# minyoungpark1/Speech-Enhancement

Hardware: AMD Instinct MI355X
Metric: utterances/sec (2 s @16 kHz) CMGAN train step (higher is better)
Workload: dtype f32 (f16x3 split); 1 GPU; cmgan generator+discriminator train step (main_gan.py train_gan loop body), batch 16/GPU, 2 s @ 16 kHz, n_fft=400 hop=100, AdamW lr 5e-4, PESQ labels supplied, kaiming-init weights; fp32 results throughout: conv and token GEMMs as scaled fp16 hi/lo splits (3 MFMAs per product, 2^-24 relative, fp32 accumulate), attention on the same scaled fp16 splits (scales from measured operand maxima), everythi; global_batch=16, parallelism=dp1

## Files before the change

speech-enhancement_amd/csrc/se_gemm.hip:

```cpp

#include "se_gemm_dev.h"


template <int BK, int PRO, bool LIN>
__global__ __launch_bounds__(256) void gemm_tap_kernel(GemmArgs g) {
  constexpr int BM = 128, BN = 64, SA = BK + 4;
  constexpr int KQ = BK / 4;
  constexpr int RPP = 256 / KQ;
  constexpr int NA = BM / RPP, NB = BN / RPP;
  __shared__ __attribute__((aligned(16))) float As[BM * SA];
  __shared__ __attribute__((aligned(16))) float Bs[BN * SA];
  __shared__ float red[4 * 64 * 2];
  __shared__ __attribute__((aligned(16))) float bias_s[64];

  const se_gemm_desc& d = g.d;
  const int tid = threadIdx.x, lane = tid & 63, wave = tid >> 6;
  const WorkId wk_ = decode_work(g.ncb, g.nouter, g.contig);
  if (wk_.outer >= g.nouter) return;
  const int b = wk_.outer / g.tiles, by = wk_.inner;
  const int Mb = d.To * d.Fo;
  const int m0 = (wk_.outer - b * g.tiles) * BM;
  const bool glu = (d.epilogue & SE_EPI_GLU) != 0;
  const int kq = tid % KQ, r0 = tid / KQ;
  constexpr bool lin = LIN;
// ... 853 lines not shown
    vr[3][ks][0] = *reinterpret_cast<const float4*>(cp + 64); vr[3][ks][1] = *reinterpret_cast<const float4*>(cp + 68);
  };
  if (k0 < ntile) {
#pragma unroll
    for (int ks = 0; ks < 4; ++ks) request(k0, ks);
  }
  int b_staged = -1;
  for (int kk = k0; kk < ntile; kk += gx) {
    const int tile = xbase + kk;
    const int b = tile / g.tiles, m0 = (tile - b * g.tiles) * 128;
    const bool ok = row_ok(kk);
    if (b != b_staged) {
      __syncthreads();
      ss_s[tid] = g.ps[(long)b * 256 + tid];
      __syncthreads();
      b_staged = b;
    }
    f32x16 acc[4];
#pragma unroll
    for (int c = 0; c < 4; ++c)
#pragma unroll
      for (int r = 0; r < 16; ++r) acc[c][r] = 0.f;
#pragma unroll
    for (int ks = 0; ks < 4; ++ks) {
      asm volatile("" ::: "memory");
      float x[8];
      {
        const float gr[8] = {vr[0][ks][0].x, vr[0][ks][0].y, vr[0][ks][0].z, vr[0][ks][0].w, vr[0][ks][1].x, vr[0][ks][1].y, vr[0][ks][1].z, vr[0][ks][1].w};
        const float fr[8] = {vr[1][ks][0].x, vr[1][ks][0].y, vr[1][ks][0].z, vr[1][ks][0].w, vr[1][ks][1].x, vr[1][ks][1].y, vr[1][ks][1].z, vr[1][ks][1].w};
        const float cg[8] = {vr[2][ks][0].x, vr[2][ks][0].y, vr[2][ks][0].z, vr[2][ks][0].w, vr[2][ks][1].x, vr[2][ks][1].y, vr[2][ks][1].z, vr[2][ks][1].w};
        const float cf[8] = {vr[3][ks][0].x, vr[3][ks][0].y, vr[3][ks][0].z, vr[3][ks][0].w, vr[3][ks][1].x, vr[3][ks][1].y, vr[3][ks][1].z, vr[3][ks][1].w};
        const float* sg = ss_s + 2 * (16 * ks + 8 * kg);
#pragma unroll
        for (int j = 0; j < 8; j += 2) {
          const float4 pg = *reinterpret_cast<const float4*>(sg + 2 * j), pf = *reinterpret_cast<const float4*>(sg + 128 + 2 * j);
          const float zg0 = fmaf(gr[j], pg.x, pg.y) + cg[j], zg1 = fmaf(gr[j + 1], pg.z, pg.w) + cg[j + 1];
          const float zf0 = fmaf(fr[j], pf.x, pf.y) + cf[j], zf1 = fmaf(fr[j + 1], pf.z, pf.w) + cf[j + 1];
          const float t0 = 1.0f - 2.0f * __builtin_amdgcn_rcpf(1.0f + __builtin_amdgcn_exp2f(2.8853900817779268f * zf0));
          const float t1 = 1.0f - 2.0f * __builtin_amdgcn_rcpf(1.0f + __builtin_amdgcn_exp2f(2.8853900817779268f * zf1));
          x[j] = ok ? sigmoidf_(zg0) * t0 : 0.f;
          x[j + 1] = ok ? sigmoidf_(zg1) * t1 : 0.f;
        }
      }
      bf16x8 af[2];
      split_planes8_h(x, sa, af);
#ifdef SE_GATE_PROJ_EARLY
      if (ks < 2) request(kk + gx, ks);
#endif
#pragma unroll
      for (int cb = 0; cb < 2; ++cb) {
        bf16x8 bf0[2], bf1[2];
#pragma unroll
        for (int pl = 0; pl < 2; ++pl) {
          bf0[pl] = *reinterpret_cast<const bf16x8*>(&Wl[(cb * 2 + pl) * PW + frag + 16 * ks]);
          bf1[pl] = *reinterpret_cast<const bf16x8*>(&Wl[(cb * 2 + pl) * PW + 32 * SW + frag + 16 * ks]);
        }
        acc[2 * cb] = mfma32_<true>(af[1], bf0[0], acc[2 * cb]); acc[2 * cb + 1] = mfma32_<true>(af[1], bf1[0], acc[2 * cb + 1]);
        acc[2 * cb] = mfma32_<true>(af[0], bf0[1], acc[2 * cb]); acc[2 * cb + 1] = mfma32_<true>(af[0], bf1[1], acc[2 * cb + 1]);
        acc[2 * cb] = mfma32_<true>(af[0], bf0[0], acc[2 * cb]); acc[2 * cb + 1] = mfma32_<true>(af[0], bf1[0], acc[2 * cb + 1]);
      }
    }
#pragma unroll
    for (int c = 0; c < 4; ++c)
#pragma unroll
      for (int r = 0; r < 16; ++r) acc[c][r] *= unscale;
#pragma unroll
    for (int cb = 0; cb < 2; ++cb) {
      gemm_epilogue_vec<false, false, true>(g, acc[2 * cb], acc[2 * cb + 1], m0, cb, b, cs, 36, 0u, 1.f, red, bias_s + 64 * cb, {}, &ymax);
      if (d.epilogue & SE_EPI_STATS) __syncthreads();
    }
#ifndef SE_GATE_PROJ_EARLY
    request(kk + gx, 0);
    request(kk + gx, 1);
#endif
    request(kk + gx, 2);
    request(kk + gx, 3);
  }
  if (g.amax_out) {
    ymax = wave_max(ymax);
    if ((threadIdx.x & 63) == 0) amax_raise_(g.amax_out, ymax);
  }
}

template <int PRO>
__global__ __launch_bounds__(512, 1) void gemm_k64_wstat_kernel(GemmArgs g) {
  constexpr int SB = 72;
  extern __shared__ __attribute__((aligned(16))) unsigned char smem_ws[];
  const se_gemm_desc& d = g.d;
  const int tid = threadIdx.x, lane = tid & 63, wave = tid >> 6;
  const int Mb = d.To * d.Fo;
  float ymax = 0.f;
  const int ncb = g.ncb, NR = ncb * 64, PB = NR * SB;
  __bf16* Bp = reinterpret_cast<__bf16*>(smem_ws);
  float* patch = reinterpret_cast<float*>(smem_ws + (size_t)2 * PB * 2);
  float* pss = patch + 8 * 32 * 36;
  float* bias_all = pss + 128;
  const bool glu = (d.epilogue & SE_EPI_GLU) != 0;
  const unsigned thr = drop_thr(d.drop_p);
  const float inv_keep = drop_inv_keep(d.drop_p);
  f16_clamp_mode_();
  const int ea = operand_sexp_(d.a_amax, d.a_sexp), ew = operand_sexp_(d.w_amax, d.w_sexp);
  const float sa = exp2i_(ea), unscale = exp2i_(-ea - ew);
  for (int i = tid; i < NR * 8; i += 512) {
    const int j = i >> 3, ch = i & 7, by = j >> 6, jl = j & 63;
    int n; bool ok;
    if (glu) { n = (jl >> 5) * (d.N / 2) + by * 32 + (jl & 31); ok = (by * 32 + (jl & 31)) < d.N / 2; }
    else { n = j; ok = n < d.N; }
    const __bf16* wp = reinterpret_cast<const __bf16*>(g.W) + ((unsigned)(ok ? n : 0) * (unsigned)d.ldw + 8 * ch);
#pragma unroll
    for (int q = 0; q < 2; ++q) {
      const uint4 w4 = *reinterpret_cast<const uint4*>(wp + (size_t)q * (size_t)d.w_planes);
      *reinterpret_cast<uint4*>(&Bp[q * PB + j * SB + 8 * ch]) = make_uint4(ok ? w4.x : 0u, ok ? w4.y : 0u, ok ? w4.z : 0u, ok ? w4.w : 0u);
    }
  }
  if (PRO == SE_PRO_LN && tid < 32) *reinterpret_cast<float4*>(&pss[4 * tid]) = *reinterpret_cast<const float4*>((tid < 16 ? g.ps : g.pb - 64) + 4 * tid);
  for (int i = tid; i < NR; i += 512) {
    const int by = i >> 6, jl = i & 63;
    int n; bool ok;
    if (glu) { n = (jl >> 5) * (d.N / 2) + by * 32 + (jl & 31); ok = (by * 32 + (jl & 31)) < d.N / 2; }
    else { n = i; ok = n < d.N; }
    bias_all[i] = ((d.epilogue & SE_EPI_BIAS) && ok) ? g.bias[n] : 0.f;
  }
  __syncthreads();
  const bool vec_ep = epilogue_vec_ok(d);
  const int kg = lane >> 5;
  const int frag = (lane & 31) * SB + 8 * kg;
  float* cs = patch + wave * 32 * 36;
  const int ntile = (Mb + 255) / 256;
  float4 v[4][2];
  float2 mr = make_float2(0.f, 0.f);
  auto request = [&](int tile) {
    const int row = tile * 256 + wave * 32 + (lane & 31);
    const long rowl = row < Mb ? row : Mb - 1;
    const float* __restrict__ ap = g.A + rowl * d.lda + d.a_off + 8 * kg;
    if (PRO == SE_PRO_LN) mr = *reinterpret_cast<const float2*>(g.rowstats + 2 * rowl);
#pragma unroll
    for (int ks = 0; ks < 4; ++ks) {
      v[ks][0] = *reinterpret_cast<const float4*>(ap + 16 * ks);
      v[ks][1] = *reinterpret_cast<const float4*>(ap + 16 * ks + 4);
    }
  };
  if ((int)blockIdx.x < ntile) request(blockIdx.x);
  for (int tile = blockIdx.x; tile < ntile; tile += gridDim.x) {
    const int m0 = tile * 256;
    const int row = m0 + wave * 32 + (lane & 31);
    const bool rok = row < Mb;
    bf16x8 af[4][2];
#pragma unroll
    for (int ks = 0; ks < 4; ++ks) {
      float x[8];
#pragma unroll
      for (int h = 0; h < 2; ++h) {
        const int c = 16 * ks + 8 * kg + 4 * h;
        float4 w = v[ks][h];
        if (PRO == SE_PRO_LN)
          w = apply_pro<PRO>(w, c, 64, mr.x, mr.y, *reinterpret_cast<const float4*>(&pss[c]), *reinterpret_cast<const float4*>(&pss[64 + c]),
                             (unsigned)row, d.pro_seed, thr, inv_keep);
        x[4 * h] = rok ? w.x : 0.f; x[4 * h + 1] = rok ? w.y : 0.f; x[4 * h + 2] = rok ? w.z : 0.f; x[4 * h + 3] = rok ? w.w : 0.f;
      }
      split_planes8_h(x, sa, af[ks]);
    }
    if (tile + (int)gridDim.x < ntile) request(tile + gridDim.x);
    for (int by = 0; by < ncb; ++by) {
      f32x16 acc0, acc1;
#pragma unroll
      for (int r = 0; r < 16; ++r) { acc0[r] = 0.f; acc1[r] = 0.f; }
      const __bf16* Bb = Bp + by * 64 * SB;
#pragma unroll
      for (int ks = 0; ks < 4; ++ks) {
        bf16x8 bf0[2], bf1[2];
#pragma unroll
        for (int pl = 0; pl < 2; ++pl) {
          bf0[pl] = *reinterpret_cast<const bf16x8*>(&Bb[pl * PB + frag + 16 * ks]);
          bf1[pl] = *reinterpret_cast<const bf16x8*>(&Bb[pl * PB + 32 * SB + frag + 16 * ks]);
        }
        acc0 = mfma32_<true>(af[ks][0], bf0[1], acc0); acc1 = mfma32_<true>(af[ks][0], bf1[1], acc1);
        acc0 = mfma32_<true>(af[ks][1], bf0[0], acc0); acc1 = mfma32_<true>(af[ks][1], bf1[0], acc1);
        acc0 = mfma32_<true>(af[ks][0], bf0[0], acc0); acc1 = mfma32_<true>(af[ks][0], bf1[0], acc1);
      }
#pragma unroll
      for (int r = 0; r < 16; ++r) { acc0[r] *= unscale; acc1[r] *= unscale; }
      if (vec_ep) gemm_epilogue_vec<false, false, true>(g, acc0, acc1, m0, by, 0, cs, 36, thr, inv_keep, nullptr, bias_all + by * 64, {}, &ymax);
      else gemm_epilogue_glu_vec(g, acc0, acc1, m0, by, 0, cs, 36, bias_all + by * 64);
    }
  }
  if (g.amax_out) {
    ymax = wave_max(ymax);
    if ((threadIdx.x & 63) == 0) amax_raise_(g.amax_out, ymax);
  }
}

__global__ void repack_kernel(const float* src, float* dst, int No, int Nt, int Ni, long so, long stt,
                              long si, int rev, int accumulate) {
  long idx = (long)blockIdx.x * blockDim.x + threadIdx.x;
  long total = (long)No * Nt * Ni;
  if (idx >= total) return;
  int i = (int)(idx % Ni);
  int t = (int)((idx / Ni) % Nt);
  int o = (int)(idx / ((long)Ni * Nt));
  int is = i, os = o;
  if (rev == 1) { int ns = Ni / 64; is = (ns - 1 - i / 64) * 64 + (i & 63); }
  if (rev == 2) { int ns = No / 64; os = (ns - 1 - o / 64) * 64 + (o & 63); }
  float v = src[os * so + is * si + t * stt];
  if (accumulate) dst[idx] += v; else dst[idx] = v;
}

__global__ void unpack_kernel(const float* src, float* dst, int No, int Nt, int Ni, long so, long stt,
                              long si, int rev, int accumulate) {
  long idx = (long)blockIdx.x * blockDim.x + threadIdx.x;
  long total = (long)No * Nt * Ni;
  if (idx >= total) return;
  int i = (int)(idx % Ni);
  int t = (int)((idx / Ni) % Nt);
  int o = (int)(idx / ((long)Ni * Nt));
  int is = i, os = o;
  if (rev == 1) { int ns = Ni / 64; is = (ns - 1 - i / 64) * 64 + (i & 63); }
  if (rev == 2) { int ns = No / 64; os = (ns - 1 - o / 64) * 64 + (o & 63); }
  float* p = &dst[os * so + is * si + t * stt];
  if (accumulate) *p += src[idx]; else *p = src[idx];
}

extern "C" int se_gemm_tap(const se_gemm_desc* d, const float* A, const float* W, const float* bias,
                           float* Y, const float* R, float* AUX, const float* rowstats,
                           const float* pro_scale, const float* pro_shift, double* stats, void* stream) {
  if (int e = check_desc(d)) return e;
  const int ep = d->epilogue;
  SE_REQUIRE(!(ep & SE_EPI_LN_BWD_), "gemm: unknown epilogue bit 1024 (use se_gemm_ln_bwd)");
  SE_REQUIRE(A && W && Y, "gemm: null operand");
  SE_REQUIRE(!(ep & SE_EPI_BIAS) || bias, "gemm: bias flag without bias");
  SE_REQUIRE(!(ep & SE_EPI_RESID) || R, "gemm: resid flag without R");
  SE_REQUIRE(!(ep & SE_EPI_SWISH_GRAD) || AUX, "gemm: swish-grad flag without AUX");
  SE_REQUIRE(!(ep & SE_EPI_STATS) || stats, "gemm: stats flag without buffer");
  if (ep & SE_EPI_ROWSTATS)
    SE_REQUIRE(AUX && d->N == 64 && d->C >= 32 && d->ntap == 1 && d->B == 1 && !(ep & (SE_EPI_GLU | SE_EPI_SHUFFLE2 | SE_EPI_SWISH_GRAD | SE_EPI_STATS)) &&
               (d->ldc & 3) == 0 && (d->c_off & 3) == 0 && (d->ldr & 3) == 0 && (d->r_off & 3) == 0,
               "gemm: SE_EPI_ROWSTATS needs a row GEMM with N == 64, AUX = [M][2] and a vector-epilogue layout");
  if (ep & SE_EPI_DELTA)
    SE_REQUIRE(AUX && R && d->N == 64 && d->C >= 32 && d->ntap == 1 && d->B == 1 &&
               !(ep & (SE_EPI_GLU | SE_EPI_SHUFFLE2 | SE_EPI_SWISH_GRAD | SE_EPI_STATS | SE_EPI_RESID | SE_EPI_ROWSTATS | SE_EPI_ACCUM | 256)) &&
               (d->ldc & 3) == 0 && (d->c_off & 3) == 0 && d->ldr >= 64 && (d->ldr & 3) == 0 && (d->r_off & 3) == 0,
               "gemm: SE_EPI_DELTA needs a row GEMM with C >= 32, N == 64, R = O [M][64], AUX = [M][4] and a vector-epilogue layout");
  SE_REQUIRE(!(ep & (SE_EPI_GLU | SE_EPI_SHUFFLE2)) || (d->N % 2) == 0, "gemm: GLU/shuffle need even N");
  SE_REQUIRE(!(ep & SE_EPI_GLU_GATE) || ((ep & SE_EPI_GLU) && AUX), "gemm: SE_EPI_GLU_GATE needs SE_EPI_GLU and AUX");
  if (d->prologue == SE_PRO_LN) SE_REQUIRE(rowstats && pro_scale && pro_shift, "gemm: LN prologue operands");
  if (d->prologue == SE_PRO_AFFINE_SWISH) SE_REQUIRE(pro_scale && pro_shift, "gemm: affine prologue operands");
  if (d->precision == 3)
    SE_REQUIRE(d->C >= 32 && (!d->w_planes || d->w_amax), "gemm: precision 3 (scaled split-fp16) needs C >= 32; pre-split planes need w_amax");
  if (d->w_planes) {
    SE_REQUIRE((d->precision == 2 || d->precision == 3) && d->C >= 32 && (d->C % 8) == 0 && (d->ldw % 8) == 0 && d->w_planes >= (long)d->N * d->ldw &&
               (d->w_planes % 8) == 0 && ((size_t)W & 15) == 0,
               "gemm: pre-split weights need precision 2, C >= 32, C, ldw and the plane stride multiples of 8, a 16-byte aligned W");
    SE_REQUIRE((long)d->w_planes * 6 < (1L << 31), "gemm: pre-split weight planes exceed 2^31 bytes");
  }
  GemmArgs g{*d, A, W, bias, Y, R, AUX, rowstats, pro_scale, pro_shift, stats, nullptr, nullptr, 0, 0, 0, 0};
  g.amax_out = d->y_amax;
  SE_REQUIRE(!d->y_amax || (!(ep & (SE_EPI_GLU | SE_EPI_SHUFFLE2 | 256)) && (d->N & 3) == 0 && (d->ldc & 3) == 0 && (d->c_off & 3) == 0 &&
                            (d->ldx & 3) == 0 && (d->x_off & 3) == 0 && (d->ldr & 3) == 0 && (d->r_off & 3) == 0),
             "gemm: y_amax needs the vector epilogue (no GLU / shuffle, 4-aligned strides)");
  const int Mb = d->To * d->Fo;
  const int ncols = (ep & SE_EPI_GLU) ? cdiv(d->N / 2, 32) : cdiv(d->N, 64);
  g.ncb = ncols;
  g.tiles = cdiv(Mb, 128);
  g.nouter = d->B * g.tiles;
  g.contig = d->ntap > 1;
  dim3 grid((unsigned)(ncols * (((long)g.nouter + 7) / 8 * 8))), block(256);
  const bool lin = d->ntap == 1 && !d->up && d->st == 1 && d->sf == 1 && d->dt[0] == 0 && d->df[0] == 0 &&
                   d->Ti == d->To && d->Fi == d->Fo;
  hipStream_t s = as_stream(stream);
  {
    const bool vec_ok = !(ep & (SE_EPI_GLU | SE_EPI_SHUFFLE2 | SE_EPI_STATS | 256)) && (d->N & 3) == 0 && (d->ldc & 3) == 0 &&
                        (d->c_off & 3) == 0 && (d->ldx & 3) == 0 && (d->x_off & 3) == 0 && (d->ldr & 3) == 0 && (d->r_off & 3) == 0;
    const bool glu_ok = (ep & SE_EPI_GLU) && !(ep & (SE_EPI_STATS | SE_EPI_SHUFFLE2 | SE_EPI_DROP | SE_EPI_RESID | SE_EPI_ACCUM |
                                                       SE_EPI_SWISH_GRAD | 256)) &&
                        (d->N & 7) == 0 && (d->ldc & 3) == 0 && (d->c_off & 3) == 0 && (d->ldx & 3) == 0 && (d->x_off & 3) == 0;
    const bool map1d = d->To == 1 && d->Ti == 1 && d->Fi == d->Fo && d->st == 1 && d->sf == 1 && !d->up;
    const bool vec_st = vec_ok || ((ep & SE_EPI_STATS) && map1d && !(ep & (SE_EPI_GLU | SE_EPI_SHUFFLE2 | SE_EPI_ROWSTATS | 256)) &&
                                   (d->N & 3) == 0 && (d->ldc & 3) == 0 && (d->c_off & 3) == 0 && (d->ldx & 3) == 0 &&
                                   (d->x_off & 3) == 0 && (d->ldr & 3) == 0 && (d->r_off & 3) == 0);
    const bool tap3 = map1d && d->ntap == 3 && d->dt[0] == 0 && d->dt[1] == 0 && d->dt[2] == 0 && d->precision == 3 && d->w_planes &&
                      d->prologue == SE_PRO_NONE && !(ep & (SE_EPI_SWISH_GRAD | SE_EPI_RESID)) && d->ldw == 192;
    const bool gate = d->prologue == SE_PRO_GATE;
    if (gate)
      SE_REQUIRE(map1d && lin && d->precision == 3 && d->w_planes && d->ldw == 64 && d->C == 64 && d->lda >= 128 && d->ldx >= 128 && (d->ldx & 3) == 0 &&
                 (d->x_off & 3) == 0 && AUX && pro_scale && !d->a_amax && vec_st && (d->w_planes % 8) == 0 &&
                 !(ep & (SE_EPI_ACCUM | SE_EPI_DROP | SE_EPI_SWISH_GRAD | SE_EPI_RESID | SE_EPI_ROWSTATS)),
                 "gemm: SE_PRO_GATE needs a 1-D row GEMM with C = 64, 128-wide A / AUX rows, scaled fp16 weight planes, a static a_sexp");
    if (map1d && (tap3 || (lin && d->precision == 3 && d->w_planes && (d->prologue == SE_PRO_NONE || gate) && d->ldw == 64)) && d->C == 64 && vec_st &&
        !(ep & (SE_EPI_ACCUM | SE_EPI_DROP | SE_EPI_SWISH_GRAD | SE_EPI_RESID | SE_EPI_ROWSTATS | SE_EPI_DELTA)) && ((long)d->B * g.tiles >= 2048 || gate) &&
        (d->w_planes % 8) == 0) {
      int ngroups = 512 / ncols < 8 ? 8 : 512 / ncols;
      if ((long)ngroups > (long)d->B * g.tiles) ngroups = d->B * g.tiles;
      ngroups = (ngroups + 7) / 8 * 8;
      const dim3 wgrid((unsigned)(ncols * ngroups));
      if (tap3) hipLaunchKernelGGL(conv1d_k64_wstat_kernel<3>, wgrid, block, 0, s, g, ngroups);
      else if (gate) {
        static const bool gate_one_wg = !(getenv("SE_GATE_PROJ_SPLIT") != nullptr);
        if (gate_one_wg && d->N == 128) {
          int ng = 512;
          if ((long)ng > (long)d->B * g.tiles) ng = d->B * g.tiles;
          ng = (ng + 7) / 8 * 8;
          hipLaunchKernelGGL(gate_proj_kernel, dim3((unsigned)ng), block, 0, s, g, ng);
        } else hipLaunchKernelGGL((conv1d_k64_wstat_kernel<1, true>), wgrid, block, 0, s, g, ngroups);
      }
      else hipLaunchKernelGGL(conv1d_k64_wstat_kernel<1>, wgrid, block, 0, s, g, ngroups);
      return se_check_launch("se_gemm_tap(W-stationary 1-D)");
    }
    if (lin && d->B == 1 && d->C == 64 && ncols >= 2 && d->precision == 3 && d->w_planes && (d->w_planes % 8) == 0 && d->ldw == 64 &&
        (d->prologue == SE_PRO_NONE || d->prologue == SE_PRO_LN) && (vec_ok || glu_ok) &&
        !(ep & (SE_EPI_ACCUM | SE_EPI_SWISH_GRAD | SE_EPI_RESID | SE_EPI_STATS | SE_EPI_DELTA)) && Mb >= 128 * 1024) {
      const size_t shw = (size_t)2 * ncols * 64 * 72 * 2 + (size_t)8 * 32 * 36 * 4 + 128 * 4 + (size_t)ncols * 64 * 4;
      if (shw <= 160 * 1024) {
        int nwg = 256;
        if (nwg > (Mb + 255) / 256) nwg = (Mb + 255) / 256;
        static unsigned raised_ws[2] = {0u, 0u};
        if (d->prologue == SE_PRO_LN) {
          SE_REQUIRE(se_raise_lds((const void*)gemm_k64_wstat_kernel<SE_PRO_LN>, 160 * 1024, &raised_ws[1]), "gemm: cannot raise the dynamic LDS limit");
          hipLaunchKernelGGL(gemm_k64_wstat_kernel<SE_PRO_LN>, dim3(nwg), dim3(512), shw, s, g);
        } else {
          SE_REQUIRE(se_raise_lds((const void*)gemm_k64_wstat_kernel<SE_PRO_NONE>, 160 * 1024, &raised_ws[0]), "gemm: cannot raise the dynamic LDS limit");
          hipLaunchKernelGGL(gemm_k64_wstat_kernel<SE_PRO_NONE>, dim3(nwg), dim3(512), shw, s, g);
        }
        return se_check_launch("se_gemm_tap(W-stationary row panel)");
      }
    }
    if ((lin || tap3) && (d->B == 1 || map1d) && d->C == 64 && (ncols >= 2 || d->prologue == SE_PRO_DROP) && (d->precision >= 1 && d->precision <= 3) && (vec_st || glu_ok) &&
        !(ep & SE_EPI_ACCUM) && !((ep & SE_EPI_SWISH_GRAD) && (ep & SE_EPI_RESID))) {
      dim3 pgrid((unsigned)(d->B * g.tiles));
      if (tap3) {
        hipLaunchKernelGGL((gemm_k64_panel_kernel<SE_PRO_NONE, 2, false, true, true, 3>), pgrid, block, 0, s, g);
        return se_check_launch("se_gemm_tap(k64 panel, 3 taps)");
      }
      SE_REQUIRE(d->precision != 3 || d->w_planes, "gemm: the scaled split-fp16 row-panel kernel reads pre-split fp16 planes");
      const bool pre2 = (ep & (SE_EPI_SWISH_GRAD | SE_EPI_RESID | SE_EPI_DELTA)) != 0;
#define LAUNCHP2(PRO, P2) do { if (d->precision == 3) hipLaunchKernelGGL((gemm_k64_panel_kernel<PRO, 2, P2, true, true>), pgrid, block, 0, s, g); \
                          else if (d->precision == 1) hipLaunchKernelGGL((gemm_k64_panel_kernel<PRO, 2, P2>), pgrid, block, 0, s, g); \
                          else if (d->w_planes) hipLaunchKernelGGL((gemm_k64_panel_kernel<PRO, 3, P2, true>), pgrid, block, 0, s, g); \
                          else hipLaunchKernelGGL((gemm_k64_panel_kernel<PRO, 3, P2>), pgrid, block, 0, s, g); } while (0)
#define LAUNCHP(PRO) do { if (pre2) LAUNCHP2(PRO, true); else LAUNCHP2(PRO, false); } while (0)
      switch (d->prologue) {
        case SE_PRO_NONE: LAUNCHP(SE_PRO_NONE); break;
        case SE_PRO_LN: LAUNCHP(SE_PRO_LN); break;
        case SE_PRO_SWISH: LAUNCHP(SE_PRO_SWISH); break;
        case SE_PRO_AFFINE_SWISH: LAUNCHP(SE_PRO_AFFINE_SWISH); break;
        case SE_PRO_SWISH_DROP: LAUNCHP(SE_PRO_SWISH_DROP); break;
        case SE_PRO_DROP: LAUNCHP(SE_PRO_DROP); break;
        default: return se_fail("gemm: unknown prologue %d", d->prologue);
      }
#undef LAUNCHP
#undef LAUNCHP2
      return se_check_launch("se_gemm_tap(k64 panel)");
    }
  }
  if ((d->precision >= 1 && d->precision <= 3) && d->C >= 32 && d->prologue == SE_PRO_NONE && !d->up && d->st == 1 && d->sf == 1 &&
      d->Ti == d->To && d->Fi == d->Fo && d->ntap >= 3 && d->ntap % 3 == 0 && !(ep & (SE_EPI_GLU | SE_EPI_DROP)) && d->Fo >= 2) {
    bool triples = getenv("SE_GEMM_NO_CONV3") == nullptr;
    if ((long)d->To * d->Fo * d->lda * 4 >= (1L << 31) || (long)d->N * d->ldw * 4 >= (1L << 31)) triples = false;
    bool fwd_order = true, rev_order = true;
    for (int t3 = 0; t3 < d->ntap && triples; t3 += 3) {
      int seen = 0;
      for (int j = 0; j < 3; ++j) {
        if (d->dt[t3 + j] != d->dt[t3] || d->df[t3 + j] < -1 || d->df[t3 + j] > 1) triples = false;
        else seen |= 1 << (d->df[t3 + j] + 1);
        if (d->df[t3 + j] != j - 1) fwd_order = false;
        if (d->df[t3 + j] != 1 - j) rev_order = false;
      }
      if (seen != 7) triples = false;
    }
    if (triples) {
      const int ord = fwd_order ? 1 : (rev_order ? 2 : 0);
      if (d->precision == 3 && d->w_planes && ord) {
        if (d->C >= 192) {
          g.tiles = cdiv(Mb, 256);
          g.nouter = d->B * g.tiles;
          dim3 grid2((unsigned)(ncols * (((long)g.nouter + 7) / 8 * 8)));
          if (ord == 1) hipLaunchKernelGGL((conv3_bf16_kernel<2, true, true, 2, 2, 1>), grid2, block, 0, s, g);
          else hipLaunchKernelGGL((conv3_bf16_kernel<2, true, true, 2, 2, 2>), grid2, block, 0, s, g);
        } else if (ord == 1) hipLaunchKernelGGL((conv3_bf16_kernel<2, true, true, 4, 1, 1>), grid, block, 0, s, g);
        else hipLaunchKernelGGL((conv3_bf16_kernel<2, true, true, 4, 1, 2>), grid, block, 0, s, g);
        return se_check_launch("se_gemm_tap(conv3)");
      }
      if (d->precision == 3) {
        if (d->w_planes && d->C >= 192) {
          g.tiles = cdiv(Mb, 256);
          g.nouter = d->B * g.tiles;
          dim3 grid2((unsigned)(ncols * (((long)g.nouter + 7) / 8 * 8)));
          hipLaunchKernelGGL((conv3_bf16_kernel<2, true, true, 2, 2>), grid2, block, 0, s, g);
        }
        else if (d->w_planes) hipLaunchKernelGGL((conv3_bf16_kernel<2, true, true, 4>), grid, block, 0, s, g);
        else hipLaunchKernelGGL((conv3_bf16_kernel<2, false, true>), grid, block, 0, s, g);
      }
      else if (d->precision == 1) hipLaunchKernelGGL((conv3_bf16_kernel<2>), grid, block, 0, s, g);
      else if (d->w_planes) hipLaunchKernelGGL((conv3_bf16_kernel<3, true>), grid, block, 0, s, g);
      else hipLaunchKernelGGL((conv3_bf16_kernel<3>), grid, block, 0, s, g);
      return se_check_launch("se_gemm_tap(conv3)");
    }
  }
  if (d->precision == 3) {
    SE_REQUIRE((d->prologue == SE_PRO_NONE || ((d->prologue == SE_PRO_DROP || d->prologue == SE_PRO_AFFINE_SWISH) && lin)) && d->w_planes,
               "gemm: precision 3 outside the triple-tap / K = 64 row-panel kernels needs pre-split fp16 planes and no prologue "
               "(row GEMMs: or the dropout / BatchNorm-Swish prologue)");
    if (d->prologue == SE_PRO_DROP) hipLaunchKernelGGL((gemm_tap_bf16x3_kernel<SE_PRO_DROP, 2, true, true, false, true>), grid, block, 0, s, g);
    else if (d->prologue == SE_PRO_AFFINE_SWISH)
      hipLaunchKernelGGL((gemm_tap_bf16x3_kernel<SE_PRO_AFFINE_SWISH, 2, true, true, false, true>), grid, block, 0, s, g);
    else if (lin) hipLaunchKernelGGL((gemm_tap_bf16x3_kernel<SE_PRO_NONE, 2, true, true, false, true>), grid, block, 0, s, g);
    else hipLaunchKernelGGL((gemm_tap_bf16x3_kernel<SE_PRO_NONE, 2, false, true, false, true>), grid, block, 0, s, g);
    return se_check_launch("se_gemm_tap(f16x3)");
  }
// ... 150 lines not shown
```

speech-enhancement_amd/csrc/se_wgrad.hip:

```cpp
#include "se_gemm_dev.h"

struct WgradArgs {
  se_gemm_desc d;
  const float* A; const float* dY; float* dW; float* dbias;
  const float* rowstats; const float* ps; const float* pb;
  long rows_per_chunk;
  int nchunks;
  int buf_ok;
};

template <int PRO>
__global__ __launch_bounds__(256) void wgrad_kernel(WgradArgs g) {
  constexpr int SY = 68;
  constexpr int MR = 64;
  __shared__ __attribute__((aligned(16))) float Ys[MR * SY];
  __shared__ __attribute__((aligned(16))) float Xs[MR * SY];
  const se_gemm_desc& d = g.d;
  const int tid = threadIdx.x, lane = tid & 63, wave = tid >> 6;
  const int ncb = (d.C + 63) / 64;
  const int nnb = (d.N + 63) / 64;
  const WorkId wk_ = decode_work(d.ntap * ncb * nnb, g.nchunks, 0);
  if (wk_.outer >= g.nchunks) return;
  const int chunk = wk_.outer, tc = wk_.inner / nnb, nb = wk_.inner - tc * nnb;
  const int tap = tc / ncb, cb = tc - tap * ncb;
// ... 1091 lines not shown
    }
    {
      float4 v0 = fix(rn[0], !XW, nq, nok, (!XW && PRO == SE_PRO_LN) ? sn[0] : make_float2(0.f, 0.f), psn, pbn, mb + 2 * nrp);
      float4 v1 = fix(rn[1], !XW, nq, nok, (!XW && PRO == SE_PRO_LN) ? sn[1] : make_float2(0.f, 0.f), psn, pbn, mb + 2 * nrp + 1);
      if (XW && do_bias) { bsum.x += v0.x + v1.x; bsum.y += v0.y + v1.y; bsum.z += v0.z + v1.z; bsum.w += v0.w + v1.w; }
      float a4[4] = {v0.x, v0.y, v0.z, v0.w}, b4[4] = {v1.x, v1.y, v1.z, v1.w};
      unsigned* cell = reinterpret_cast<unsigned*>(&Ns[((nrp >> 2) * NARROW) * 8 + 2 * (nrp & 3)]);
      const int tq = tid & 15;
      if constexpr (F16) {
#pragma unroll
        for (int j = 0; j < 4; ++j) {
          const float ya = a4[j] * s_narrow, yb = b4[j] * s_narrow;
          const unsigned w = pk_f16_(ya, yb);
          const f16x2_ hh = __builtin_bit_cast(f16x2_, w);
          const int pc = (16 * j + ((tq + 4 * j) & 15)) * 8;
          cell[pc / 2] = w;
          cell[(NPLN + pc) / 2] = pk_f16_(ya - (float)hh[0], yb - (float)hh[1]);
        }
      } else {
#pragma unroll
        for (int q = 0; q < 3; ++q)
#pragma unroll
          for (int j = 0; j < 4; ++j) {
            const unsigned w = pk_bf16_(a4[j], b4[j]);
            cell[(q * NPLN + (16 * j + ((tq + 4 * j) & 15)) * 8) / 2] = w;
            if (q < 2) { a4[j] -= __builtin_bit_cast(float, w << 16); b4[j] -= __builtin_bit_cast(float, w & 0xffff0000u); }
          }
      }
    }
    __syncthreads();
    if (mb + MR < mend) load_tiles(mb + MR);
    if (active) {
#pragma unroll
      for (int s = 0; s < 2; ++s) {
        bf16x8 af[2][NP], bf[2][NP];
#pragma unroll
        for (int t = 0; t < 2; ++t)
#pragma unroll
          for (int q = 0; q < NP; ++q) {
            af[t][q] = *reinterpret_cast<const bf16x8*>(abase + q * APL + 2 * s * AOC + aoff[t]);
            bf[t][q] = *reinterpret_cast<const bf16x8*>(bbase + q * BPL + 2 * s * BOC + boff[t]);
          }
#pragma unroll
        for (int ord = NP - 1; ord >= 0; --ord)
#pragma unroll
          for (int qa = 0; qa <= ord; ++qa)
#pragma unroll
            for (int a = 0; a < 2; ++a)
#pragma unroll
              for (int b = 0; b < 2; ++b)
                acc[a][b] = mfma32_<F16>(af[a][qa], bf[b][ord - qa], acc[a][b]);
      }
    }
    __syncthreads();
  }
  __builtin_amdgcn_s_waitcnt(0x0F70);
  const int wn = XW ? 0 : wave, wc = XW ? wave : 0;
#pragma unroll
  for (int a = 0; a < 2; ++a)
#pragma unroll
    for (int b = 0; b < 2; ++b) {
      const int c = (wc * 2 + b) * 32 + l31;
#pragma unroll
      for (int r = 0; r < 16; ++r) {
        const int n = (wn * 2 + a) * 32 + (r & 3) + 8 * (r >> 2) + 4 * half;
        if (n < d.N && c < d.C) atomicAdd(&g.dW[(long)n * d.ldw + c], d.alpha * unscale * acc[a][b][r]);
      }
    }
  if (do_bias) {
    float* red = reinterpret_cast<float*>(Ws);
    constexpr int NG = XW ? 16 : 4, NC = XW ? NARROW : WIDE;
    const int grp = XW ? nrp : wave, c0 = XW ? nq : wq;
    *reinterpret_cast<float4*>(&red[grp * NC + c0]) = bsum;
    __syncthreads();
    if (tid < NC && tid < d.N) {
      float s_ = 0.f;
#pragma unroll
      for (int r = 0; r < NG; ++r) s_ += red[r * NC + tid];
      atomicAdd(&g.dbias[tid], d.alpha * s_);
    }
  }
}

template <int SH>
static int launch_wgrad_lin_f16(const se_gemm_desc* d, const WgradArgs& g, dim3 grid, hipStream_t s) {
  const dim3 block(256);
  switch (d->prologue) {
    case SE_PRO_NONE: hipLaunchKernelGGL((wgrad_lin_bf16_kernel<SE_PRO_NONE, SH, true>), grid, block, 0, s, g); break;
    case SE_PRO_LN: hipLaunchKernelGGL((wgrad_lin_bf16_kernel<SE_PRO_LN, SH, true>), grid, block, 0, s, g); break;
    case SE_PRO_SWISH: hipLaunchKernelGGL((wgrad_lin_bf16_kernel<SE_PRO_SWISH, SH, true>), grid, block, 0, s, g); break;
    case SE_PRO_AFFINE_SWISH: hipLaunchKernelGGL((wgrad_lin_bf16_kernel<SE_PRO_AFFINE_SWISH, SH, true>), grid, block, 0, s, g); break;
    case SE_PRO_SWISH_DROP: hipLaunchKernelGGL((wgrad_lin_bf16_kernel<SE_PRO_SWISH_DROP, SH, true>), grid, block, 0, s, g); break;
    default: return se_fail("wgrad: no scaled split-fp16 kernel for prologue %d", d->prologue);
  }
  return se_check_launch("se_gemm_tap_wgrad(lin f16x3)");
}

template <int SH>
static int launch_wgrad_lin_bf16(const se_gemm_desc* d, const WgradArgs& g, dim3 grid, hipStream_t s) {
  const dim3 block(256);
  switch (d->prologue) {
    case SE_PRO_NONE: hipLaunchKernelGGL((wgrad_lin_bf16_kernel<SE_PRO_NONE, SH>), grid, block, 0, s, g); break;
    case SE_PRO_LN: hipLaunchKernelGGL((wgrad_lin_bf16_kernel<SE_PRO_LN, SH>), grid, block, 0, s, g); break;
    case SE_PRO_SWISH: hipLaunchKernelGGL((wgrad_lin_bf16_kernel<SE_PRO_SWISH, SH>), grid, block, 0, s, g); break;
    case SE_PRO_AFFINE_SWISH: hipLaunchKernelGGL((wgrad_lin_bf16_kernel<SE_PRO_AFFINE_SWISH, SH>), grid, block, 0, s, g); break;
    case SE_PRO_SWISH_DROP: hipLaunchKernelGGL((wgrad_lin_bf16_kernel<SE_PRO_SWISH_DROP, SH>), grid, block, 0, s, g); break;
    case SE_PRO_DROP: hipLaunchKernelGGL((wgrad_lin_bf16_kernel<SE_PRO_DROP, SH>), grid, block, 0, s, g); break;
    default: return se_fail("wgrad: unknown prologue %d", d->prologue);
  }
  return se_check_launch("se_gemm_tap_wgrad(lin bf16x6)");
}

static thread_local int g_wgrad_kind = 0;
extern "C" int se_gemm_tap_wgrad_last_kind(void) { return g_wgrad_kind; }

extern "C" int se_gemm_tap_wgrad(const se_gemm_desc* d, const float* A, const float* dY, float* dW,
                                 float* dbias, const float* rowstats, const float* pro_scale,
                                 const float* pro_shift, int chunks, void* stream) {
  if (int e = check_desc(d)) return e;
  SE_REQUIRE(A && dY && dW, "wgrad: null operand");
  SE_REQUIRE((d->N % 4) == 0 && (d->ldc % 4) == 0 && (d->c_off % 4) == 0, "wgrad: N/ldc/c_off must be multiples of 4");
  if (d->prologue == SE_PRO_LN) SE_REQUIRE(rowstats && pro_scale && pro_shift, "wgrad: LN prologue operands");
  if (d->prologue == SE_PRO_AFFINE_SWISH) SE_REQUIRE(pro_scale && pro_shift, "wgrad: affine prologue operands");
  const long Mtot = (long)d->B * d->To * d->Fo;
  if (chunks < 1) chunks = 1;
  long rpc = (Mtot + chunks - 1) / chunks;
  rpc = ((rpc + 63) / 64) * 64;
  chunks = (int)((Mtot + rpc - 1) / rpc);
  WgradArgs g{*d, A, dY, dW, dbias, rowstats, pro_scale, pro_shift, rpc, chunks, 0};
  g.buf_ok = ((Mtot - 1) * d->lda + d->C) * 4 < 4294967280L && ((Mtot - 1) * d->ldc + d->N) * 4 < 4294967280L;
  dim3 grid((unsigned)((long)d->ntap * cdiv(d->C, 64) * cdiv(d->N, 64) * ((chunks + 7) / 8 * 8))), block(256);
  hipStream_t s = as_stream(stream);
  if (d->prologue == SE_PRO_NONE && !(d->epilogue & SE_EPI_DROP) && !d->up && d->st == 1 && d->sf == 1 &&
      d->Ti == d->To && d->Fi == d->Fo && d->ntap >= 3 && d->ntap % 3 == 0 && d->Fo >= 2 && d->To * d->Fo >= 64 &&
      getenv("SE_GEMM_NO_CONV3") == nullptr) {
    bool triples = true, ordered = true;
    for (int t3 = 0; t3 < d->ntap && triples; t3 += 3) {
      int seen = 0;
      for (int j = 0; j < 3; ++j) {
        if (d->dt[t3 + j] != d->dt[t3] || d->df[t3 + j] < -1 || d->df[t3 + j] > 1) triples = false;
        else seen |= 1 << (d->df[t3 + j] + 1);
        if (d->df[t3 + j] != j - 1) ordered = false;
      }
      if (seen != 7) triples = false;
    }
    if (triples && (d->precision == 0 || d->Fo > 66)) {
      dim3 g3((unsigned)((long)(d->ntap / 3) * cdiv(d->C, 64) * cdiv(d->N, 64) * ((chunks + 7) / 8 * 8)));
      if (d->precision == 3 && ordered && d->C >= 128 && g.buf_ok) {
        dim3 g3w((unsigned)((long)(d->ntap / 3) * cdiv(d->C, 128) * cdiv(d->N, 64) * ((chunks + 7) / 8 * 8)));
        hipLaunchKernelGGL(wgrad3w_f16_kernel, g3w, block, 0, s, g);
      }
      else if (d->precision == 3 && ordered) hipLaunchKernelGGL((wgrad3_bf16_kernel<2, true, true>), g3, block, 0, s, g);
      else if (d->precision == 3) hipLaunchKernelGGL((wgrad3_bf16_kernel<2, true>), g3, block, 0, s, g);
      else if (d->precision == 1) hipLaunchKernelGGL(wgrad3_bf16_kernel<2>, g3, block, 0, s, g);
      else if (d->precision == 2) hipLaunchKernelGGL(wgrad3_bf16_kernel<3>, g3, block, 0, s, g);
      else hipLaunchKernelGGL(wgrad3_kernel, g3, block, 0, s, g);
      g_wgrad_kind = 16 | (d->precision & 3);
      return se_check_launch("se_gemm_tap_wgrad(conv3)");
    }
  }
  const bool want_f16 = d->precision == 3;
  se_gemm_desc dfb;
  if (d->precision == 3) { dfb = *d; dfb.precision = 2; d = &dfb; }
  const bool lin = d->ntap == 1 && d->B == 1 && !d->up && d->st == 1 && d->sf == 1 && d->dt[0] == 0 && d->df[0] == 0 &&
                   d->Ti == d->To && d->Fi == d->Fo;
  if (lin && (d->precision == 0 || d->precision == 2) && (d->C % 4) == 0 && (d->lda % 4) == 0 && (d->a_off % 4) == 0 &&
      getenv("SE_WGRAD_NO_LIN") == nullptr) {
    int shape = 0;
    if (d->C <= 64 && d->N > 192 && d->N <= 256) shape = 1;
    else if (d->N <= 64 && d->C > 128 && d->C <= 256) shape = 2;
    const bool f16_pro = d->prologue == SE_PRO_NONE || d->prologue == SE_PRO_LN || d->prologue == SE_PRO_SWISH ||
                         d->prologue == SE_PRO_AFFINE_SWISH || d->prologue == SE_PRO_SWISH_DROP;
    if (want_f16 && f16_pro && !shape) {
      if (d->C <= 64 && d->N <= 256) shape = 1;
      else if (d->N <= 64 && d->C <= 256) shape = 2;
    }
    if (shape && d->precision == 2) {
      long rl = (Mtot + 511) / 512;
      if (rl < 256) rl = 256;
      rl = ((rl + 31) / 32) * 32;
      const int nch = (int)((Mtot + rl - 1) / rl);
      WgradArgs gl{*d, A, dY, dW, dbias, rowstats, pro_scale, pro_shift, rl, nch};
      g_wgrad_kind = 32 | ((want_f16 && f16_pro) ? 3 : 2);
      if (want_f16 && f16_pro)
        return shape == 1 ? launch_wgrad_lin_f16<1>(d, gl, dim3((unsigned)nch), s) : launch_wgrad_lin_f16<2>(d, gl, dim3((unsigned)nch), s);
      return shape == 1 ? launch_wgrad_lin_bf16<1>(d, gl, dim3((unsigned)nch), s) : launch_wgrad_lin_bf16<2>(d, gl, dim3((unsigned)nch), s);
    }
    if (shape) {
      long rl = (Mtot + 767) / 768;
      if (rl < 256) rl = 256;
      rl = ((rl + 31) / 32) * 32;
      const int nch = (int)((Mtot + rl - 1) / rl);
      WgradArgs gl{*d, A, dY, dW, dbias, rowstats, pro_scale, pro_shift, rl, nch};
      const dim3 gg((unsigned)nch);
      g_wgrad_kind = 32;
      if (shape == 1) return launch_wgrad_lin<4, 2, 2>(d, gl, gg, s);
      return launch_wgrad_lin<1, 2, 2>(d, gl, gg, s);
    }
  }
  if (d->precision == 1) {
    switch (d->prologue) {
      case SE_PRO_NONE: hipLaunchKernelGGL((wgrad_bf16_kernel<SE_PRO_NONE, 2>), grid, block, 0, s, g); break;
      case SE_PRO_LN: hipLaunchKernelGGL((wgrad_bf16_kernel<SE_PRO_LN, 2>), grid, block, 0, s, g); break;
      case SE_PRO_SWISH: hipLaunchKernelGGL((wgrad_bf16_kernel<SE_PRO_SWISH, 2>), grid, block, 0, s, g); break;
      case SE_PRO_AFFINE_SWISH: hipLaunchKernelGGL((wgrad_bf16_kernel<SE_PRO_AFFINE_SWISH, 2>), grid, block, 0, s, g); break;
      case SE_PRO_SWISH_DROP: hipLaunchKernelGGL((wgrad_bf16_kernel<SE_PRO_SWISH_DROP, 2>), grid, block, 0, s, g); break;
      case SE_PRO_DROP: hipLaunchKernelGGL((wgrad_bf16_kernel<SE_PRO_DROP, 2>), grid, block, 0, s, g); break;
      default: return se_fail("wgrad: unknown prologue %d", d->prologue);
    }
    g_wgrad_kind = d->precision;
    return se_check_launch("se_gemm_tap_wgrad(bf16)");
  }
  switch (d->prologue) {
    case SE_PRO_NONE: hipLaunchKernelGGL((wgrad_kernel<SE_PRO_NONE>), grid, block, 0, s, g); break;
    case SE_PRO_LN: hipLaunchKernelGGL((wgrad_kernel<SE_PRO_LN>), grid, block, 0, s, g); break;
    case SE_PRO_SWISH: hipLaunchKernelGGL((wgrad_kernel<SE_PRO_SWISH>), grid, block, 0, s, g); break;
    case SE_PRO_AFFINE_SWISH: hipLaunchKernelGGL((wgrad_kernel<SE_PRO_AFFINE_SWISH>), grid, block, 0, s, g); break;
    case SE_PRO_SWISH_DROP: hipLaunchKernelGGL((wgrad_kernel<SE_PRO_SWISH_DROP>), grid, block, 0, s, g); break;
    case SE_PRO_DROP: hipLaunchKernelGGL((wgrad_kernel<SE_PRO_DROP>), grid, block, 0, s, g); break;
    default: return se_fail("wgrad: unknown prologue %d", d->prologue);
  }
  g_wgrad_kind = 0;
  return se_check_launch("se_gemm_tap_wgrad");
}
```

Before: 304.9 utterances/sec.

## Add weight-stationary N=64 forward path with delta epilogue and narrow f16x3 wgrad kernel

Extends the weight-stationary K=64 row-panel GEMM to single-column-block (N=64) cases with dropout prologue or a delta epilogue, prefetching the residual/delta operand alongside the A rows. Adds a dedicated narrow weight-gradient kernel for N<=64, C<=128 that splits dY and X into fp16 hi/lo planes in LDS per wave and accumulates with MFMAs, then reduces across waves before atomics. Both target the many small 64-channel linear layers, aiming to cut the overhead of the generic tile kernels. The new paths add template variants and register pressure, and the wgrad path now bypasses the previous shape-specific kernels for these sizes.

```diff
diff --git a/speech-enhancement_amd/csrc/se_gemm.hip b/speech-enhancement_amd/csrc/se_gemm.hip
--- a/speech-enhancement_amd/csrc/se_gemm.hip
+++ b/speech-enhancement_amd/csrc/se_gemm.hip
@@ -959,8 +959,8 @@
   }
 }
 
-template <int PRO>
-__global__ __launch_bounds__(512, 1) void gemm_k64_wstat_kernel(GemmArgs g) {
+template <int PRO, bool DLT>
+static __device__ __forceinline__ void gemm_k64_wstat_body(const GemmArgs& g) {
   constexpr int SB = 72;
   extern __shared__ __attribute__((aligned(16))) unsigned char smem_ws[];
   const se_gemm_desc& d = g.d;
@@ -1005,6 +1005,7 @@
   float* cs = patch + wave * 32 * 36;
   const int ntile = (Mb + 255) / 256;
   float4 v[4][2];
+  float4 pre_next[8], pre[8];
   float2 mr = make_float2(0.f, 0.f);
   auto request = [&](int tile) {
     const int row = tile * 256 + wave * 32 + (lane & 31);
@@ -1015,6 +1016,16 @@
     for (int ks = 0; ks < 4; ++ks) {
       v[ks][0] = *reinterpret_cast<const float4*>(ap + 16 * ks);
       v[ks][1] = *reinterpret_cast<const float4*>(ap + 16 * ks + 4);
+    }
+    if (DLT) {
+#pragma unroll
+      for (int nt = 0; nt < 2; ++nt)
+#pragma unroll
+        for (int i = 0; i < 4; ++i) {
+          const int prow = tile * 256 + wave * 32 + (lane >> 3) + 8 * i;
+          const long prl = prow < Mb ? prow : Mb - 1;
+          pre_next[nt * 4 + i] = *reinterpret_cast<const float4*>(g.R + prl * d.ldr + d.r_off + nt * 32 + (lane & 7) * 4);
+        }
     }
   };
   if ((int)blockIdx.x < ntile) request(blockIdx.x);
@@ -1033,9 +1044,15 @@
         if (PRO == SE_PRO_LN)
           w = apply_pro<PRO>(w, c, 64, mr.x, mr.y, *reinterpret_cast<const float4*>(&pss[c]), *reinterpret_cast<const float4*>(&pss[64 + c]),
                              (unsigned)row, d.pro_seed, thr, inv_keep);
+        else if (PRO == SE_PRO_DROP)
+          w = apply_pro<PRO>(w, c, 64, 0.f, 0.f, make_float4(0.f, 0.f, 0.f, 0.f), make_float4(0.f, 0.f, 0.f, 0.f), (unsigned)row, d.pro_seed, thr, inv_keep);
         x[4 * h] = rok ? w.x : 0.f; x[4 * h + 1] = rok ? w.y : 0.f; x[4 * h + 2] = rok ? w.z : 0.f; x[4 * h + 3] = rok ? w.w : 0.f;
       }
       split_planes8_h(x, sa, af[ks]);
+    }
+    if (DLT) {
+#pragma unroll
+      for (int i = 0; i < 8; ++i) pre[i] = pre_next[i];
     }
     if (tile + (int)gridDim.x < ntile) request(tile + gridDim.x);
     for (int by = 0; by < ncb; ++by) {
@@ -1057,7 +1074,8 @@
       }
 #pragma unroll
       for (int r = 0; r < 16; ++r) { acc0[r] *= unscale; acc1[r] *= unscale; }
-      if (vec_ep) gemm_epilogue_vec<false, false, true>(g, acc0, acc1, m0, by, 0, cs, 36, thr, inv_keep, nullptr, bias_all + by * 64, {}, &ymax);
+      if constexpr (DLT) gemm_epilogue_vec<true, false, true, true>(g, acc0, acc1, m0, by, 0, cs, 36, thr, inv_keep, nullptr, bias_all + by * 64, pre, &ymax);
+      else if (vec_ep) gemm_epilogue_vec<false, false, true>(g, acc0, acc1, m0, by, 0, cs, 36, thr, inv_keep, nullptr, bias_all + by * 64, {}, &ymax);
       else gemm_epilogue_glu_vec(g, acc0, acc1, m0, by, 0, cs, 36, bias_all + by * 64);
     }
   }
@@ -1066,6 +1084,11 @@
     if ((threadIdx.x & 63) == 0) amax_raise_(g.amax_out, ymax);
   }
 }
+
+template <int PRO>
+__global__ __launch_bounds__(512, 1) void gemm_k64_wstat_kernel(GemmArgs g) { gemm_k64_wstat_body<PRO, false>(g); }
+template <int PRO>
+__global__ __launch_bounds__(512, 1) void gemm_k64_wstat_delta_kernel(GemmArgs g) { gemm_k64_wstat_body<PRO, true>(g); }
 
 __global__ void repack_kernel(const float* src, float* dst, int No, int Nt, int Ni, long so, long stt,
                               long si, int rev, int accumulate) {
@@ -1200,6 +1223,20 @@
         return se_check_launch("se_gemm_tap(W-stationary row panel)");
       }
     }
+    if (lin && d->B == 1 && d->C == 64 && d->N == 64 && ncols == 1 && d->precision == 3 && d->w_planes && (d->w_planes % 8) == 0 && d->ldw == 64 &&
+        (d->prologue == SE_PRO_NONE || d->prologue == SE_PRO_DROP) && (d->prologue == SE_PRO_DROP || (ep & SE_EPI_DELTA)) && vec_ok &&
+        !(ep & (SE_EPI_ACCUM | SE_EPI_SWISH_GRAD | SE_EPI_RESID | SE_EPI_STATS | SE_EPI_ROWSTATS)) && Mb >= 128 * 1024 &&
+        getenv("SE_GEMM_NO_WSTAT_N64") == nullptr) {
+      const size_t shw = (size_t)2 * 64 * 72 * 2 + (size_t)8 * 32 * 36 * 4 + 128 * 4 + (size_t)64 * 4;
+      int nwg = 256;
+      if (nwg > (Mb + 255) / 256) nwg = (Mb + 255) / 256;
+      const bool drop = d->prologue == SE_PRO_DROP;
+      if (ep & SE_EPI_DELTA) {
+        if (drop) hipLaunchKernelGGL(gemm_k64_wstat_delta_kernel<SE_PRO_DROP>, dim3(nwg), dim3(512), shw, s, g);
+        else hipLaunchKernelGGL(gemm_k64_wstat_delta_kernel<SE_PRO_NONE>, dim3(nwg), dim3(512), shw, s, g);
+      } else hipLaunchKernelGGL(gemm_k64_wstat_kernel<SE_PRO_DROP>, dim3(nwg), dim3(512), shw, s, g);
+      return se_check_launch("se_gemm_tap(W-stationary row panel, N = 64)");
+    }
     if ((lin || tap3) && (d->B == 1 || map1d) && d->C == 64 && (ncols >= 2 || d->prologue == SE_PRO_DROP) && (d->precision >= 1 && d->precision <= 3) && (vec_st || glu_ok) &&
         !(ep & SE_EPI_ACCUM) && !((ep & SE_EPI_SWISH_GRAD) && (ep & SE_EPI_RESID))) {
       dim3 pgrid((unsigned)(d->B * g.tiles));
diff --git a/speech-enhancement_amd/csrc/se_wgrad.hip b/speech-enhancement_amd/csrc/se_wgrad.hip
--- a/speech-enhancement_amd/csrc/se_wgrad.hip
+++ b/speech-enhancement_amd/csrc/se_wgrad.hip
@@ -1197,6 +1197,185 @@
   }
 }
 
+template <int PRO>
+__global__ __launch_bounds__(256, 2) void wgrad_lin_narrow_f16_kernel(WgradArgs g) {
+  constexpr int IMG = 4 * 64 * 8;
+  __shared__ __attribute__((aligned(16))) __bf16 St[4 * 4 * IMG];
+  __shared__ __attribute__((aligned(16))) float bred[16 * 64];
+  const se_gemm_desc& d = g.d;
+  const int tid = threadIdx.x, lane = tid & 63, wave = tid >> 6;
+  const int half = lane >> 5, l31 = lane & 31, sub = lane >> 4, tq = lane & 15, cq = tq * 4;
+  const long Mtot = (long)d.To * d.Fo;
+  const long mbeg = (long)blockIdx.x * g.rows_per_chunk;
+  long mend = mbeg + g.rows_per_chunk;
+  if (mend > Mtot) mend = Mtot;
+  const bool wide_c = d.C > 64;
+  const int rblk = wide_c ? wave >> 1 : wave, cblk = wide_c ? wave & 1 : 0, step = wide_c ? 64 : 128;
+  const int cx = 64 * cblk + cq;
+  const bool yok = cq < d.N, xok = cx < d.C;
+  const float* __restrict__ Yg = g.dY + d.c_off + (yok ? cq : 0);
+  const float* __restrict__ Xg = g.A + d.a_off + (xok ? cx : 0);
+  const long ldy = d.ldc, ldx = d.lda;
+  const unsigned thr = drop_thr(d.drop_p);
+  const float inv_keep = drop_inv_keep(d.drop_p);
+  const bool dy_drop = (d.epilogue & SE_EPI_DROP) != 0;
+  const bool do_bias = g.dbias != nullptr;
+  f16_clamp_mode_();
+  const int ex = operand_sexp_(d.a_amax, d.a_sexp), ey = operand_sexp_(d.w_amax, d.w_sexp);
+  const float s_x = exp2i_(ex), s_y = exp2i_(ey), unscale = exp2i_(-ex - ey);
+
+  f32x16 acc[2][2];
+#pragma unroll
+  for (int a = 0; a < 2; ++a)
+#pragma unroll
+    for (int b = 0; b < 2; ++b)
+#pragma unroll
+      for (int r = 0; r < 16; ++r) acc[a][b][r] = 0.f;
+  float4 bsum = make_float4(0.f, 0.f, 0.f, 0.f);
+  float4 ry[8], rx[8];
+  float2 sx[8];
+  float4 ps4 = make_float4(0.f, 0.f, 0.f, 0.f), pb4 = ps4;
+  load_pro_vec<PRO>(g.ps, g.pb, cx, xok, ps4, pb4);
+  const int r0 = 32 * rblk + sub;
+  auto load_y = [&](long mbase) {
+#pragma unroll
+    for (int i = 0; i < 8; ++i) {
+      long mg = mbase + r0 + 4 * i;
+      mg = mg < mend ? mg : mend - 1;
+      ry[i] = *reinterpret_cast<const float4*>(Yg + mg * ldy);
+    }
+  };
+  auto load_x = [&](long mbase) {
+#pragma unroll
+    for (int i = 0; i < 8; ++i) {
+      long mg = mbase + r0 + 4 * i;
+      mg = mg < mend ? mg : mend - 1;
+      rx[i] = *reinterpret_cast<const float4*>(Xg + mg * ldx);
+      if (PRO == SE_PRO_LN) sx[i] = *reinterpret_cast<const float2*>(g.rowstats + 2 * mg);
+    }
+  };
+  if (mbeg < mend) { load_y(mbeg); load_x(mbeg); }
+  __bf16* img = St + wave * 4 * IMG;
+  auto swn = [](int c) { return 16 * (c & 3) + (((c >> 2) + 4 * (c & 3)) & 15); };
+  const int f0 = swn(l31) * 8, f1 = swn(32 + l31) * 8;
+  const int foff[2] = {f0, f1};
+  for (long mb = mbeg; mb < mend; mb += step) {
+    {
+      float4 v[8];
+#pragma unroll
+      for (int i = 0; i < 8; ++i) {
+        const long mg = mb + r0 + 4 * i;
+        const bool live = yok && mg < mend;
+        float4 u = ry[i];
+        if (dy_drop) {
+          const float4 d4 = drop_scale4(d.epi_seed, (unsigned)(mg * d.N + cq), thr, inv_keep);
+          u.x *= d4.x; u.y *= d4.y; u.z *= d4.z; u.w *= d4.w;
+        }
+        v[i] = make_float4(live ? u.x : 0.f, live ? u.y : 0.f, live ? u.z : 0.f, live ? u.w : 0.f);
+        if (do_bias) { bsum.x += v[i].x; bsum.y += v[i].y; bsum.z += v[i].z; bsum.w += v[i].w; }
+      }
+#pragma unroll
+      for (int j = 0; j < 4; ++j) {
+        const int cell = (sub * 64 + 16 * j + ((tq + 4 * j) & 15)) * 8;
+        float x[8];
+        bf16x8 pl[2];
+#pragma unroll
+        for (int i = 0; i < 8; ++i) x[i] = j == 0 ? v[i].x : (j == 1 ? v[i].y : (j == 2 ? v[i].z : v[i].w));
+        split_planes8_h(x, s_y, pl);
+        *reinterpret_cast<bf16x8*>(&img[cell]) = pl[0];
+        *reinterpret_cast<bf16x8*>(&img[IMG + cell]) = pl[1];
+      }
+    }
+    if (mb + step < mend) load_y(mb + step);
+    {
+      float4 v[8];
+#pragma unroll
+      for (int i = 0; i < 8; ++i) {
+        const long mg = mb + r0 + 4 * i;
+        const bool live = xok && mg < mend;
+        float4 u = rx[i];
+        if (PRO != SE_PRO_NONE)
+          u = apply_pro<PRO>(u, cx, d.C, PRO == SE_PRO_LN ? sx[i].x : 0.f, PRO == SE_PRO_LN ? sx[i].y : 0.f, ps4, pb4, mg, d.pro_seed, thr, inv_keep);
+        v[i] = make_float4(live ? u.x : 0.f, live ? u.y : 0.f, live ? u.z : 0.f, live ? u.w : 0.f);
+      }
+#pragma unroll
+      for (int j = 0; j < 4; ++j) {
+        const int cell = (sub * 64 + 16 * j + ((tq + 4 * j) & 15)) * 8;
+        float x[8];
+        bf16x8 pl[2];
+#pragma unroll
+        for (int i = 0; i < 8; ++i) x[i] = j == 0 ? v[i].x : (j == 1 ? v[i].y : (j == 2 ? v[i].z : v[i].w));
+        split_planes8_h(x, s_x, pl);
+        *reinterpret_cast<bf16x8*>(&img[2 * IMG + cell]) = pl[0];
+        *reinterpret_cast<bf16x8*>(&img[3 * IMG + cell]) = pl[1];
+      }
+    }
+    if (mb + step < mend) load_x(mb + step);
+#pragma unroll
+    for (int s = 0; s < 2; ++s) {
+      bf16x8 af[2][2], bf[2][2];
+#pragma unroll
+      for (int t = 0; t < 2; ++t)
+#pragma unroll
+        for (int q = 0; q < 2; ++q) {
+          af[t][q] = *reinterpret_cast<const bf16x8*>(&img[q * IMG + (2 * s + half) * 64 * 8 + foff[t]]);
+          bf[t][q] = *reinterpret_cast<const bf16x8*>(&img[(2 + q) * IMG + (2 * s + half) * 64 * 8 + foff[t]]);
+        }
+#pragma unroll
+      for (int ord = 1; ord >= 0; --ord)
+#pragma unroll
+        for (int qa = 0; qa <= ord; ++qa)
+#pragma unroll
+          for (int a = 0; a < 2; ++a)
+#pragma unroll
+            for (int b = 0; b < 2; ++b)
+              acc[a][b] = mfma32_<true>(af[a][qa], bf[b][ord - qa], acc[a][b]);
+    }
+  }
+  __builtin_amdgcn_s_waitcnt(0x0F70);
+  float* part = reinterpret_cast<float*>(St);
+#pragma unroll
+  for (int a = 0; a < 2; ++a)
+#pragma unroll
+    for (int b = 0; b < 2; ++b)
+#pragma unroll
+      for (int r = 0; r < 16; ++r)
+        part[wave * 4096 + (a * 32 + (r & 3) + 8 * (r >> 2) + 4 * half) * 64 + b * 32 + l31] = acc[a][b][r];
+  if (do_bias)
+    *reinterpret_cast<float4*>(&bred[(wave * 4 + sub) * 64 + cq]) = cblk == 0 ? bsum : make_float4(0.f, 0.f, 0.f, 0.f);
+  __syncthreads();
+  const float sc = d.alpha * unscale;
+  const int ncb = wide_c ? 2 : 1;
+  for (int cb = 0; cb < ncb; ++cb)
+#pragma unroll
+    for (int k = 0; k < 16; ++k) {
+      const int e = tid + 256 * k, n = e >> 6, c = 64 * cb + (e & 63);
+      float s_;
+      if (wide_c) s_ = part[cb * 4096 + e] + part[(2 + cb) * 4096 + e];
+      else s_ = (part[e] + part[4096 + e]) + (part[8192 + e] + part[12288 + e]);
+      if (n < d.N && c < d.C) atomicAdd(&g.dW[(long)n * d.ldw + c], sc * s_);
+    }
+  if (do_bias && tid < 64 && tid < d.N) {
+    float s_ = 0.f;
+#pragma unroll
+    for (int r = 0; r < 16; ++r) s_ += bred[r * 64 + tid];
+    atomicAdd(&g.dbias[tid], d.alpha * s_);
+  }
+}
+
+static int launch_wgrad_lin_narrow_f16(const se_gemm_desc* d, const WgradArgs& g, dim3 grid, hipStream_t s) {
+  const dim3 block(256);
+  switch (d->prologue) {
+    case SE_PRO_NONE: hipLaunchKernelGGL((wgrad_lin_narrow_f16_kernel<SE_PRO_NONE>), grid, block, 0, s, g); break;
+    case SE_PRO_LN: hipLaunchKernelGGL((wgrad_lin_narrow_f16_kernel<SE_PRO_LN>), grid, block, 0, s, g); break;
+    case SE_PRO_SWISH: hipLaunchKernelGGL((wgrad_lin_narrow_f16_kernel<SE_PRO_SWISH>), grid, block, 0, s, g); break;
+    case SE_PRO_AFFINE_SWISH: hipLaunchKernelGGL((wgrad_lin_narrow_f16_kernel<SE_PRO_AFFINE_SWISH>), grid, block, 0, s, g); break;
+    case SE_PRO_SWISH_DROP: hipLaunchKernelGGL((wgrad_lin_narrow_f16_kernel<SE_PRO_SWISH_DROP>), grid, block, 0, s, g); break;
+    default: return se_fail("wgrad: no scaled split-fp16 kernel for prologue %d", d->prologue);
+  }
+  return se_check_launch("se_gemm_tap_wgrad(lin narrow f16x3)");
+}
+
 template <int SH>
 static int launch_wgrad_lin_f16(const se_gemm_desc* d, const WgradArgs& g, dim3 grid, hipStream_t s) {
   const dim3 block(256);
@@ -1290,6 +1469,15 @@
       if (d->C <= 64 && d->N <= 256) shape = 1;
       else if (d->N <= 64 && d->C <= 256) shape = 2;
     }
+    if (want_f16 && f16_pro && d->N <= 64 && d->C <= 128 && getenv("SE_WGRAD_NO_NARROW") == nullptr) {
+      long rl = (Mtot + 511) / 512;
+      if (rl < 256) rl = 256;
+      rl = ((rl + 127) / 128) * 128;
+      const int nch = (int)((Mtot + rl - 1) / rl);
+      WgradArgs gl{*d, A, dY, dW, dbias, rowstats, pro_scale, pro_shift, rl, nch};
+      g_wgrad_kind = 32 | 3;
+      return launch_wgrad_lin_narrow_f16(d, gl, dim3((unsigned)nch), s);
+    }
     if (shape && d->precision == 2) {
       long rl = (Mtot + 511) / 512;
       if (rl < 256) rl = 256;
```

Result: no change. 307.8 utterances/sec, median of 6 (+1.0%).
